# mahdi-slh/DeformContact

Hardware: AMD Instinct MI355X
Metric: M edges/sec fwd+bwd, everyday-deform batch=32 per GPU (encoder hot path) (higher is better)
Workload: dtype f32 (hops, storage, accumulate); wide dense blocks fp16x2-split operands (3 fp16 MFMA products, fp32 accumulate), narrow ones bf16x3-split (6 products); 1 GPU; everyday-deform synthetic, B=32 sample pairs per GPU: soft 32x(1024 v, 6132 e) + rigid 32x(762 v, 4560 e); TAGConv encoder 2 layers/branch, hidden 256, K=3 (configs[1]); edges_per_gpu_step=342144, global_batch=32, settle_steps=150, hipgraph=True, two_stream_branches=True, merged_branches=False, segmented_adjacency_build=True, parallelism=dp1

## Files before the change

### deformcontact_amd/_lib.py

```python
from __future__ import annotations

import ctypes
import os
from ctypes import POINTER, c_char_p, c_float, c_int, c_int32, c_int64, c_void_p

_HERE = os.path.dirname(os.path.abspath(__file__))
SO_PATH = os.path.join(_HERE, "libdeformcontact_hip.so")

_lib = None

_vp = c_void_p
_SIGNATURES = {
    "dc_version": (c_int, []),
    "dc_last_error": (c_char_p, []),
    "dc_stream_capture_id": (c_int64, [_vp]),
    "dc_csr_workspace_bytes": (c_int64, [c_int64, c_int64]),
    "dc_csr_build": (c_int, [_vp, c_int64, c_int64, c_int, c_int, _vp, _vp, _vp, _vp, _vp, _vp,
                             _vp, c_int64, _vp]),
    "dc_graph_workspace_bytes": (c_int64, [c_int64, c_int64]),
    "dc_graph_build": (c_int, [_vp, c_int64, c_int64, c_int, _vp, _vp, _vp, _vp, _vp, _vp, _vp, _vp,
                               _vp, _vp, c_int64, _vp]),
    "dc_graph_build_parts": (c_int, [POINTER(_vp), POINTER(c_int64), POINTER(c_int64), POINTER(c_int64), c_int,
                                     c_int64, c_int, _vp, _vp, _vp, _vp, _vp, _vp, _vp, _vp, _vp, _vp, c_int64,
                                     _vp]),
# ... 12 lines not shown
                                             _vp]),
    "dc_attn_flash_fwd": (c_int, [_vp, c_int64, _vp, _vp, _vp, _vp, _vp, c_int64, c_int64, c_int64, c_int64, _vp,
                                  c_int64, _vp, _vp]),
    "dc_hop_chain_max_nodes": (c_int64, []),
    "dc_hop_chain_lds_request": (c_int64, []),
    "dc_hop_chain_f32": (c_int, [_vp, _vp, _vp, _vp, c_int64, POINTER(c_int64), c_int, _vp, c_int64, c_int64, c_int64,
                                 c_int, c_int, c_int, _vp, c_int, _vp]),
    "dc_spmm_f32_bias_act": (c_int, [_vp, _vp, _vp, _vp, c_int64, _vp, c_int, _vp, c_int64, c_int64, c_int64, _vp]),
    "dc_colsum_workspace_bytes": (c_int64, [c_int64, c_int64, c_int]),
    "dc_mask_colsum_f32": (c_int, [_vp, c_int64, _vp, c_int64, _vp, c_int64, c_int64, c_int64, _vp, c_int64, _vp, c_int,
                                   _vp]),
    "dc_gat_alpha_fwd": (c_int, [_vp, c_int64, _vp, _vp, _vp, _vp, c_int64, c_int64, _vp]),
    "dc_gat_alpha_bwd": (c_int, [_vp, c_int64, _vp, _vp, _vp, _vp, _vp, c_int64, c_int64, c_int64, _vp, c_int64, _vp, _vp,
                                 c_int, _vp]),
    "dc_spmm_f32_pack": (c_int, [_vp, _vp, _vp, _vp, c_int64, _vp, c_int64, c_int64, c_int64, c_int64, c_int64, _vp]),
    "dc_spmm_f32_window": (c_int, [_vp, _vp, _vp, _vp, c_int64, _vp, c_int64, _vp, c_int64, c_int64,
                                   c_int64, c_int64, _vp]),
    "dc_spmm_f32_rowmax_window": (c_int, [_vp, _vp, _vp, _vp, c_int64, _vp, c_int64, _vp, c_int64, c_int64,
                                          c_int64, _vp, c_int, c_int64, _vp]),
    "dc_tag_grouped_weight_prep": (c_int, [POINTER(_vp), c_int, c_int, c_int64, c_int64, POINTER(_vp),
                                           POINTER(_vp), POINTER(_vp), POINTER(_vp), _vp]),
    "dc_tag_grouped_fwd_h2p": (c_int, [_vp, c_int64, c_int, POINTER(c_int64), POINTER(c_int64), c_int64,
                                       POINTER(_vp), POINTER(_vp), c_int, _vp, c_int64, c_int64, c_int64, _vp,
                                       POINTER(_vp), _vp]),
    "dc_tag_grouped_mask_grad": (c_int, [POINTER(_vp), POINTER(c_int64), c_int, POINTER(c_int64),
                                         POINTER(c_int64), c_int64, _vp, c_int64, _vp, c_int64, c_int64, _vp,
                                         _vp, _vp]),
    "dc_tag_grouped_bwd_dw_workspace_bytes": (c_int64, [POINTER(c_int64), c_int, c_int64, c_int64, c_int]),
    "dc_tag_grouped_bwd_dw_h2": (c_int, [_vp, c_int64, POINTER(_vp), POINTER(c_int64), c_int, c_int,
                                         POINTER(c_int64), POINTER(c_int64), c_int64, POINTER(_vp),
# ... 187 lines not shown
```

### deformcontact_amd/csrc/dc_dense.h

```cpp
#pragma once
#include <stdlib.h>

#include "dc_common.h"

namespace dc {

constexpr int BK = 16;
constexpr int LDK = BK + 4;
constexpr int BN = 128;
constexpr int kMaxSeg = DC_MAX_SEG;

using f32x16 = __attribute__((ext_vector_type(16))) float;
using f16x4 = __attribute__((ext_vector_type(4))) _Float16;
using f16x8 = __attribute__((ext_vector_type(8))) _Float16;
using bf16x4 = __attribute__((ext_vector_type(4))) __bf16;
using bf16x8 = __attribute__((ext_vector_type(8))) __bf16;
using s16x4 = __attribute__((ext_vector_type(4))) short;
typedef __attribute__((address_space(3))) s16x4 lds_s16x4;

__device__ __forceinline__ int lds_row_swz(int row) { return ((row >> 1) & 7) ^ ((row & 1) << 1); }

__device__ __forceinline__ void split1(float x, __bf16 &hi, __bf16 &mid, __bf16 &lo) {
    hi = (__bf16)x;
    const float r = x - (float)hi;
    mid = (__bf16)r;
    const float r2 = r - (float)mid;
    lo = (__bf16)r2;
}

__device__ __forceinline__ void split4_h2(const float4 &v, f16x4 &h, f16x4 &l) {
    const float x[4] = {v.x, v.y, v.z, v.w};
#pragma unroll
    for (int i = 0; i < 4; ++i) {
        const _Float16 a = (_Float16)x[i];
        h[i] = a;
        l[i] = (_Float16)(x[i] - (float)a);
    }
}

template <int ROWB>
__device__ __forceinline__ bf16x8 tr_read(const char *a) {
    const s16x4 lo4 = __builtin_amdgcn_ds_read_tr16_b64_v4i16((lds_s16x4 *)(uintptr_t)(a));
// ... 227 lines not shown
```

### deformcontact_amd/csrc/dc_dense_narrow.hip

```cpp
#include "dc_dense.h"

#ifndef DC_NARROW_ABL
#define DC_NARROW_ABL 0
#endif

namespace dc {

struct NarrowParams {
    const float *x;
    int64_t ld;
    const float *w[kMaxSeg];
    int nseg, fi;
    const float *bias;
    float *out;
    int64_t ldo, N;
    int relu, ntiles;
};

constexpr int kNarrowFo = 256;


template <int KS, int MB>
__global__ void __launch_bounds__(256)
k_fwd_narrow(NarrowParams p) {
    constexpr int TR = 32 * MB;
    constexpr int SROWA = KS * 96 + 16;
    constexpr int PPR = 4 * KS;
    constexpr int TP = TR * PPR, NV = (TP + 255) / 256;
    constexpr int KP = 16 * KS;
    constexpr int kOffStage = ((TR * SROWA + 1023) / 1024) * 1024;
    constexpr int kLdsTiles = kOffStage + TR * 1024, kLdsW = kNarrowFo * (KP + 4) * 4;
    __shared__ __attribute__((aligned(1024))) char lds[kLdsTiles > kLdsW ? kLdsTiles : kLdsW];
    char *const sA = lds;
    float *const so = reinterpret_cast<float *>(lds + kOffStage);
// ... 5 lines not shown
        const int64_t row0 = (int64_t)t * TR;
#pragma unroll
        for (int j = 0; j < NV; ++j) {
            const int q = (int)threadIdx.x + 256 * j;
            if (TP % 256 != 0 && q >= TP) continue;
            const int r = q / PPR, c4 = q - r * PPR;
            int64_t row = row0 + r;
            row = row < p.N ? row : p.N - 1;
            if (DC_NARROW_ABL & 8) xv[j] = f32x4{(float)row, 1.f, 2.f, 3.f};
            else xv[j] = *reinterpret_cast<const f32x4 *>(p.x + row * p.ld + 4 * c4);
        }
    };
    int t = blockIdx.x;
    if (t < p.ntiles) load_tile(t);

    constexpr int WROW = KP + 4;
    {
        float *wi = reinterpret_cast<float *>(lds);
        const int width = p.nseg * p.fi, per4 = kNarrowFo * p.fi / 4;
        constexpr int MAXQ = 8;
        f32x4 wv[kMaxSeg][MAXQ];
#pragma unroll
        for (int s = 0; s < kMaxSeg; ++s)
#pragma unroll
            for (int j = 0; j < MAXQ; ++j) {
                const int q = (int)threadIdx.x + 256 * j;
                if (!(DC_NARROW_ABL & 2) && s < p.nseg && q < per4) wv[s][j] = *reinterpret_cast<const f32x4 *>(p.w[s] + 4 * q);
            }
#pragma unroll
        for (int s = 0; s < kMaxSeg; ++s)
#pragma unroll
            for (int j = 0; j < MAXQ; ++j) {
                const int q = (int)threadIdx.x + 256 * j;
                if (!(DC_NARROW_ABL & 2) && s < p.nseg && q < per4) {
                    int o = (4 * q) / p.fi, f = 4 * q - o * p.fi;
#pragma unroll
                    for (int i = 0; i < 4; ++i) {
                        wi[o * WROW + s * p.fi + f] = wv[s][j][i];
                        if (++f == p.fi) f = 0, ++o;
                    }
                }
            }
        const int padw = KP - width;
        for (int e = threadIdx.x; e < kNarrowFo * padw; e += 256) {
            const int o = e / padw, f = e - o * padw;
            wi[o * WROW + width + f] = 0.f;
        }
    }
    __syncthreads();
    bf16x8 fb[2][KS][3];
#pragma unroll
    for (int nb = 0; nb < 2; ++nb) {
        const float *wr = reinterpret_cast<const float *>(lds) + (64 * wid + 32 * nb + c) * WROW + 8 * h;
#pragma unroll
        for (int ks = 0; ks < KS; ++ks) {
            const f32x4 v0 = *reinterpret_cast<const f32x4 *>(wr + 16 * ks);
            const f32x4 v1 = *reinterpret_cast<const f32x4 *>(wr + 16 * ks + 4);
#pragma unroll
            for (int j = 0; j < 8; ++j) {
                __bf16 hi, mid, lo;
                split1(j < 4 ? v0[j] : v1[j - 4], hi, mid, lo);
                fb[nb][ks][0][j] = hi, fb[nb][ks][1][j] = mid, fb[nb][ks][2][j] = lo;
            }
        }
    }
    __syncthreads();
    float bcol[2];
#pragma unroll
    for (int nb = 0; nb < 2; ++nb) bcol[nb] = p.bias ? p.bias[64 * wid + 32 * nb + c] : 0.f;
    const bool relu = p.relu != 0;

    auto store_tile = [&]() {
#pragma unroll
        for (int j = 0; j < NV; ++j) {
            const int q = (int)threadIdx.x + 256 * j;
            if (TP % 256 != 0 && q >= TP) continue;
            const int r = q / PPR, c4 = q - r * PPR;
            bf16x4 hi, mid, lo;
#pragma unroll
            for (int i = 0; i < 4; ++i) {
                __bf16 a, b, d;
// ... 72 lines not shown
    NarrowParams p = p0;
    p.ntiles = (int)((p.N + 31) / 32);
    const unsigned grid = (unsigned)(p.ntiles < 256 ? p.ntiles : 256);
    DC_LAUNCH((k_fwd_narrow<KS, 1>), dim3(grid), dim3(256), 0, hs, p);
}

}

using namespace dc;

extern "C" int dc_tag_linear_fwd_narrow_ok(int64_t fi, int nseg, int64_t wpad, int64_t Fo) {
    return (Fo == kNarrowFo && nseg >= 1 && nseg <= kMaxSeg && fi >= 1 && fi <= 32 && nseg * fi <= wpad &&
            (wpad == 96 || wpad == 112 || wpad == 128)) ? 1 : 0;
}

extern "C" int dc_tag_linear_fwd_narrow(const float *slab, int64_t ld, const float *const *ws, int nseg, int64_t fi,
                                        const float *bias, int relu, float *out, int64_t ldo, int64_t N, int64_t wpad,
                                        int64_t Fo, dc_stream_t stream) {
    DC_REQUIRE(dc_tag_linear_fwd_narrow_ok(fi, nseg, wpad, Fo),
               "dc_tag_linear_fwd_narrow: needs Fo = 256, a padded reduction of 96 / 112 / 128 >= nseg * fi (got Fo=%lld wpad=%lld "
               "nseg=%d fi=%lld)", (long long)Fo, (long long)wpad, nseg, (long long)fi);
    DC_REQUIRE(N >= 0, "dc_tag_linear_fwd_narrow: negative N");
    if (N == 0) return DC_OK;
    DC_REQUIRE(slab && ws && out && ld >= wpad && ldo >= Fo, "dc_tag_linear_fwd_narrow: null pointer / short leading dimension");
    DC_REQUIRE(ld % 4 == 0 && ldo % 4 == 0 && ((uintptr_t)slab & 15) == 0 && ((uintptr_t)out & 15) == 0,
               "dc_tag_linear_fwd_narrow: rows of the slab and of the output must be 16-byte aligned");
    DC_REQUIRE(N < ((int64_t)1 << 31) - 64, "dc_tag_linear_fwd_narrow: too many rows");
    NarrowParams p{};
    p.x = slab, p.ld = ld, p.nseg = nseg, p.fi = (int)fi, p.bias = bias, p.out = out, p.ldo = ldo, p.N = N, p.relu = relu;
    for (int s = 0; s < nseg; ++s) {
        DC_REQUIRE(ws[s], "dc_tag_linear_fwd_narrow: null weight segment %d", s);
        p.w[s] = ws[s];
    }
    hipStream_t hs = (hipStream_t)stream;
    switch (wpad) {
    case 96: narrow_launch<6>(p, hs); break;
    case 112: narrow_launch<7>(p, hs); break;
    default: narrow_launch<8>(p, hs); break;
    }
    return check_launch("dc_tag_linear_fwd_narrow");
}
```

### deformcontact_amd/csrc/dc_spmm.hip

```cpp
#include <stdlib.h>

#include "dc_common.h"

#pragma clang fp contract(off)

namespace dc {

template <int VEC> struct Vec;
template <> struct Vec<1> { using T = float; };
template <> struct Vec<4> { using T = float4; };

__device__ __forceinline__ float vzero(float) { return 0.0f; }
__device__ __forceinline__ float4 vzero(float4) { return make_float4(0.f, 0.f, 0.f, 0.f); }

__device__ __forceinline__ void vaxpy(float &acc, float w, float v) {
    const float m = w * v;
    acc = acc + m;
}
__device__ __forceinline__ void vaxpy(float4 &acc, float w, const float4 &v) {
    const float mx = w * v.x, my = w * v.y, mz = w * v.z, mw = w * v.w;
    acc.x = acc.x + mx;
    acc.y = acc.y + my;
    acc.z = acc.z + mz;
    acc.w = acc.w + mw;
// ... 101 lines not shown
        ww[0] = row_share_f<0>(my_w), ww[1] = row_share_f<1>(my_w), ww[2] = row_share_f<2>(my_w);
        ww[3] = row_share_f<3>(my_w), ww[4] = row_share_f<4>(my_w), ww[5] = row_share_f<5>(my_w);
        ww[6] = row_share_f<6>(my_w), ww[7] = row_share_f<7>(my_w);
    } else {
        const bool mine = sub < 8 && p + sub < end;
        const int my_s = mine ? other[p + sub] : 0;
        const float my_w = mine ? (w ? w[p + sub] : 1.0f) : 0.0f;
#pragma unroll
        for (int j = 0; j < 8; ++j) {
            s[j] = __shfl(my_s, j, L);
            ww[j] = __shfl(my_w, j, L);
        }
    }
}

template <int VEC, int L, int U>
__global__ void __launch_bounds__(256)
k_spmm_sub(const int32_t *__restrict__ ptr, const int32_t *__restrict__ other,
           const float *__restrict__ w, const float *__restrict__ x, int64_t ldx,
           const float *addend, int64_t ldadd, float *y, int64_t ldy,
           int64_t N, int F, int src_off, float *self_dst = nullptr, int pad_beg = 0, int pad_end = 0) {
    using V = typename Vec<VEC>::T;
    constexpr int kRows = 256 / L;
    const unsigned lb = xcd_remap(blockIdx.x, gridDim.x);
    const int64_t row = (int64_t)lb * kRows + threadIdx.x / L;
    if (row >= N) return;
    const int sub = threadIdx.x % L;
    const int beg = ptr[row], end = ptr[row + 1];
    if (self_dst) {
        for (int c = sub; c < F; c += L) self_dst[row * ldy + c] = x[row * ldx + c];
        for (int c = pad_beg + sub; c < pad_end; c += L) self_dst[row * ldy + c] = 0.f;
    }

    for (int c0 = 0; c0 < F; c0 += L * VEC) {
        const int c = c0 + sub * VEC;
        const bool act = c < F;
        V acc = (addend && act) ? *reinterpret_cast<const V *>(addend + row * ldadd + c) : vzero(V{});
        for (int p = beg; p < end; p += U) {
            int s[U];
// ... 14 lines not shown
                const bool ok = act && p + j < end;
                v[j] = ok ? *reinterpret_cast<const V *>(x + (int64_t)(s[j] - src_off) * ldx + c) : vzero(V{});
            }
#pragma unroll
            for (int j = 0; j < U; ++j)
                if (p + j < end) vaxpy(acc, ww[j], v[j]);
        }
        if (act) *reinterpret_cast<V *>(y + row * ldy + c) = acc;
    }
}

template <int VEC, int L, int U>
static void launch_sub(const int32_t *ptr, const int32_t *other, const float *w, const float *x,
                       int64_t ldx, const float *addend, int64_t ldadd, float *y, int64_t ldy,
                       int64_t N, int F, int src_off, hipStream_t stream, float *self_dst = nullptr,
                       int pad_beg = 0, int pad_end = 0) {
    constexpr int kRows = 256 / L;
    const unsigned grid = (unsigned)((N + kRows - 1) / kRows);
    DC_LAUNCH((k_spmm_sub<VEC, L, U>), dim3(grid), dim3(256), 0, stream, ptr, other, w, x,
                       ldx, addend, ldadd, y, ldy, N, F, src_off, self_dst, pad_beg, pad_end);
}

static inline bool aligned16(const void *p) { return ((uintptr_t)p & 15) == 0; }

__device__ __forceinline__ float bf16_to_f32(uint16_t h) { return __uint_as_float((uint32_t)h << 16); }

struct Bf16x8 { uint4 q; };
__device__ __forceinline__ void unpack8(const uint4 &q, float (&v)[8]) {
    const uint32_t d[4] = {q.x, q.y, q.z, q.w};
#pragma unroll
    for (int i = 0; i < 4; ++i) {
        v[2 * i] = __uint_as_float(d[i] << 16);
        v[2 * i + 1] = __uint_as_float(d[i] & 0xffff0000u);
    }
}
// ... 300 lines not shown
    DC_REQUIRE(ptr && x && y, "dc_spmm_f32_bias_act: null ptr/x/y");
    DC_REQUIRE(N < (int64_t)INT32_MAX / 4 && F < (1 << 24) && ldx >= F && ldy >= F && x != y,
               "dc_spmm_f32_bias_act: bad sizes / aliasing");
    const bool vec4 = (F % 4 == 0) && (ldx % 4 == 0) && (ldy % 4 == 0) && aligned16(x) && aligned16(y) &&
                      (!bias || aligned16(bias));
    const unsigned grid = (unsigned)((N + 3) / 4);
    if (vec4)
        DC_LAUNCH((k_spmm_wave<4, 8, false, true>), dim3(grid), dim3(256), 0, stream, ptr, other, w, x, ldx, nullptr,
                  (int64_t)0, y, ldy, N, (int)F, nullptr, 0, 0, bias, relu);
    else
        DC_LAUNCH((k_spmm_wave<1, 8, false, true>), dim3(grid), dim3(256), 0, stream, ptr, other, w, x, ldx, nullptr,
                  (int64_t)0, y, ldy, N, (int)F, nullptr, 0, 0, bias, relu);
    return check_launch("dc_spmm_f32_bias_act");
}

extern "C" int dc_spmm_f32_pack(const int32_t *ptr, const int32_t *other, const float *w, const float *x,
                                int64_t ldx, float *slab, int64_t lds, int64_t N, int64_t F, int64_t width,
                                int64_t wpad, dc_stream_t stream_) {
    hipStream_t stream = (hipStream_t)stream_;
    DC_REQUIRE(N >= 0 && F >= 1 && F <= 32, "dc_spmm_f32_pack: rows of 1..32 floats (got F=%lld)", (long long)F);
    if (N == 0) return DC_OK;
    DC_REQUIRE(ptr && x && slab && (other || true), "dc_spmm_f32_pack: null pointer");
    DC_REQUIRE(N < (int64_t)INT32_MAX / 8 && ldx >= F && width >= 2 * F && wpad >= width && lds >= wpad,
               "dc_spmm_f32_pack: needs ldx >= F, width >= 2 F (block 1 exists), wpad >= width, lds >= wpad");
    DC_REQUIRE((const void *)x != (const void *)slab, "dc_spmm_f32_pack: the slab must not alias x");
    float *y = slab + F;
    if (F > 16)
        launch_sub<1, 32, 8>(ptr, other, w, x, ldx, nullptr, 0, y, lds, N, (int)F, 0, stream, slab, (int)width, (int)wpad);
    else if (F > 8)
        launch_sub<1, 16, 8>(ptr, other, w, x, ldx, nullptr, 0, y, lds, N, (int)F, 0, stream, slab, (int)width, (int)wpad);
    else
        launch_sub<1, 8, 8>(ptr, other, w, x, ldx, nullptr, 0, y, lds, N, (int)F, 0, stream, slab, (int)width, (int)wpad);
    return check_launch("dc_spmm_f32_pack");
}

extern "C" int dc_spmm_f32_window(const int32_t *ptr, const int32_t *other, const float *w,
                                  const float *x, int64_t ldx, const float *addend, int64_t ldadd,
                                  float *y, int64_t ldy, int64_t N, int64_t F, int64_t row_offset,
                                  dc_stream_t stream) {
    DC_REQUIRE(row_offset >= 0 && row_offset < (int64_t)INT32_MAX, "dc_spmm_f32_window: bad row_offset");
    return spmm_f32_impl(ptr, other, w, x, ldx, addend, ldadd, y, ldy, N, F, (int)row_offset, stream);
}

extern "C" int dc_spmm_bf16(const int32_t *ptr, const int32_t *other, const float *w,
                            const uint16_t *x, int64_t ldx, const void *addend, int64_t ldadd,
                            void *y, int64_t ldy, int64_t N, int64_t F, int y_is_f32,
                            dc_stream_t stream_) {
    hipStream_t stream = (hipStream_t)stream_;
// ... 60 lines not shown
```

### deformcontact_amd/ops.py

```python
from __future__ import annotations

import ctypes
import os
from typing import List, Optional

import torch

from . import _lib
from .deferred import resolve
from .graph import GraphIndex, SortedAdjacency, _require_cuda, capture_id, current_stream_ptr


def _rowmajor(t: torch.Tensor, what: str, dtypes=(torch.float32,)) -> int:
    if t.dim() != 2 or t.dtype not in dtypes:
        raise ValueError(f"{what}: expected a 2-D tensor of {dtypes}, got {tuple(t.shape)} {t.dtype}")
    if t.size(1) > 1 and t.stride(1) != 1:
        raise ValueError(f"{what}: innermost dimension must be contiguous")
    return t.stride(0) if t.size(0) > 1 else max(t.stride(0), t.size(1))


def _vp_array(ptrs):
    return (ctypes.c_void_p * len(ptrs))(*ptrs)


# ... 204 lines not shown
        return slab, rowmax
    return None


def _hop_cache_put(g, key, x, slab, rowmax, dev):
    cache = g.__dict__.setdefault("_hop_cache", {})
    if key not in cache:
        while len(cache) >= _HOP_CACHE_ENTRIES:
            cache.pop(next(iter(cache)))
    cache[key] = (slab, rowmax, capture_id(dev), x, x._version)


FUSED_PACK = os.environ.get("DC_FUSED_PACK", "1") != "0"


def _build_input_slab(g: GraphIndex, x: torch.Tensor, k: int, want_rowmax: bool, into=None):
    n, fi = x.shape
    concat, width, wpad = tag_slab_geometry(fi, k)
    dev = x.device
    slab = into[0] if into is not None else _alloc_slab(n, wpad, dev)
    xin = x if (x.dim() == 2 and x.stride(1) == 1) else x.contiguous()
    adj = g.fwd if (g is not None and k >= 1) else None
    if (FUSED_PACK and adj is not None and not want_rowmax and fi <= 32 and not adj.row_offset and g.normalize
            and adj.ptr.numel() == n + 1):
        _lib.check(_lib.lib().dc_spmm_f32_pack(adj.ptr.data_ptr(), adj.other.data_ptr(), adj.w.data_ptr(),
                                               xin.data_ptr(), xin.stride(0), slab.data_ptr(), slab.stride(0), n, fi,
                                               width, wpad, current_stream_ptr(dev)), "dc_spmm_f32_pack")
        for j in range(1, k):
            hop(adj, slab[:, j * fi:(j + 1) * fi], out=slab[:, (j + 1) * fi:(j + 2) * fi], weighted=True)
        return slab, None
    _lib.check(_lib.lib().dc_tag_pack_input(xin.data_ptr(), xin.stride(0), slab.data_ptr(), slab.stride(0), n,
                                            fi, width, wpad, current_stream_ptr(dev)),
               "dc_tag_pack_input")
    rowmax = None
    if want_rowmax:
        rowmax = into[1] if into is not None else torch.empty(n, dtype=torch.float32, device=dev)
    chained_hops(g, slab, fi, k, backward=False, rowmax=rowmax)
    return slab, rowmax


def _tag_uses_h2(fi: int, k: int, fo: Optional[int] = None) -> bool:
    concat, _, wpad = tag_slab_geometry(fi, k)
# ... 103 lines not shown
        return "fp32"
    if _tag_uses_h2(fi, k, None if six else fo):
        return "h2"
    if not tag_slab_geometry(fi, k)[0]:
        return "split"
    return "narrow" if (NARROW_FWD and DENSE_PRODUCTS == 6 and narrow_ok) else "concat"


def _dense_operands(slab: torch.Tensor, fi: int, k: int, concat: bool):
    ld = slab.stride(0)
    if concat:
        return [slab], [ld], slab.size(1), 1
    return [slab[:, j * fi:(j + 1) * fi] for j in range(k + 1)], [ld] * (k + 1), fi, k + 1


def _tag_slab(g, x: torch.Tensor, weights, h2: bool, need_x: bool):
    n, fi = x.shape
    k = len(weights) - 1
    dev = x.device
    wpad = tag_slab_geometry(fi, k)[2]
    slab = _as_slab_block0(x, n, fi, wpad)
    if slab is None and k == 0 and wpad == fi and x.is_contiguous() and x.data_ptr() % 16 == 0:
        slab = x
    rowmax = prepped = None
    if slab is None:
        key = None
        if HOP_CACHE and g is not None and k >= 1 and not need_x:
            key = _hop_cache_key(x, k, wpad, h2)
            hit = _hop_cache_get(g, key, x, dev)
            if hit is not None:
                slab, rowmax = hit
        if slab is None:
            slab, rowmax = _build_input_slab(g, x, k, h2)
            if key is not None:
                _hop_cache_put(g, key, x, slab, rowmax, dev)
    else:
        rowmax = torch.empty(n, dtype=torch.float32, device=dev) if h2 else None
        zeroed = False
        if h2 and g is not None and hop_chain_eligible(g, g.fwd, slab, fi, k):
            fo = weights[0].size(0)
            prepped = _h2_weight_prep(_lib.lib(), [w.contiguous() for w in weights], k, fo, fi,
                                      need_x and fo % 16 == 0, dev, current_stream_ptr(dev), zero=rowmax)
            zeroed = True
        chained_hops(g, slab, fi, k, backward=False, rowmax=rowmax, rowmax_zeroed=zeroed)
    if h2 and k == 0:
        rowmax = rowabsmax(slab)
    return slab, rowmax, prepped

# ... 143 lines not shown
            raise NotImplementedError(f"TAGConv K={k} > {MAX_SEG - 1} is not supported by the fused dense block")
        dev = x.device
        L = _lib.lib()
        st = current_stream_ptr(dev)
        six = next_geom is SIX_PRODUCTS
        if six:
            next_geom = None
        ctx.empty = n == 0
        if ctx.empty:
            ctx.fi, ctx.has_bias = fi, bias is not None
            ctx.save_for_backward(*weights)
            return _tag_out_buffer(next_geom, n, fo, dev)
        concat, width, wpad = tag_slab_geometry(fi, k)
        path = _dense_path(fi, k, fo, six, concat and bool(L.dc_tag_linear_fwd_narrow_ok(fi, k + 1, wpad, fo)))
        need_x = ctx.needs_input_grad[1]
        slab, rowmax, prepped = _tag_slab(g, x, weights, path == "h2", need_x)
        ws = [w.contiguous() for w in weights]
        if concat and path != "narrow":
            ws = [_pack_weights(ws, fo, fi, wpad, st)]
        out = _tag_out_buffer(next_geom, n, fo, dev)
        ldo = out.stride(0)
        b = bias.contiguous() if bias is not None else None
        wt = wt_rowmax = None
        if path == "h2":
            if prepped is None:
                prepped = _h2_weight_prep(L, ws, k, fo, fi, need_x and fo % 16 == 0, dev, st)
            wmax, wimg, wt, wt_rowmax = prepped
            rc = L.dc_tag_linear_fwd_h2p(slab.data_ptr(), slab.stride(0), wimg.data_ptr(), _ptr(b), int(relu),
                                         out.data_ptr(), ldo, n, width, fo, rowmax.data_ptr(), wmax.data_ptr(),
                                         None, 0, st)
        elif path == "narrow":
            rc = L.dc_tag_linear_fwd_narrow(slab.data_ptr(), slab.stride(0), _ptr_array(ws), k + 1, fi, _ptr(b),
                                            int(relu), out.data_ptr(), ldo, n, wpad, fo, st)
        else:
            xs, ldxs, fi_eff, nseg = _dense_operands(slab, fi, k, concat)
            args = (_ptr_array(xs), _i64_array(ldxs), _ptr_array(ws), nseg, _ptr(b), int(relu), out.data_ptr(), ldo,
                    n, fi_eff, fo)
            rc = L.dc_tag_linear_fwd(*args, st) if path == "fp32" else L.dc_tag_linear_fwd_split(*args, DENSE_PRODUCTS, st)
        _lib.check(rc, "dc_tag_linear_fwd")
        ctx.g, ctx.k, ctx.fi, ctx.fo, ctx.has_bias, ctx.relu, ctx.concat, ctx.path = \
            g, k, fi, fo, bias is not None, relu, concat, path
        ctx.params, ctx.bias_param = weights, bias
        ctx.save_for_backward(slab, out if relu else None, rowmax, wt, wt_rowmax, *ws)
        return out

    @staticmethod
    def backward(ctx, gout):
        if ctx.empty:
# ... 1365 lines not shown
```

### include/deformcontact.h

```cpp
#ifndef DEFORMCONTACT_H
#define DEFORMCONTACT_H

#include <stdint.h>

#ifdef __cplusplus
extern "C" {
#endif

#define DC_OK 0
#define DC_EINVAL (-1)
#define DC_ELAUNCH (-2)
#define DC_EWORKSPACE (-3)

typedef void *dc_stream_t;

#define DC_MAX_PARTS 4
#define DC_MAX_GROUPS 4
#define DC_GROUP_ALIGN 256

int dc_version(void);
const char *dc_last_error(void);
int64_t dc_stream_capture_id(dc_stream_t stream);

int64_t dc_csr_workspace_bytes(int64_t E, int64_t N);
// ... 51 lines not shown
int64_t dc_neighbors_compact_workspace_bytes(int64_t ny);
int dc_neighbors_compact(const int32_t *nbr, int cap, const int32_t *counts, int64_t ny, int query_row,
                         int64_t *edge_index, int64_t num_edges, void *workspace, int64_t workspace_bytes,
                         dc_stream_t stream);

int dc_hash_i64(const int64_t *v, int64_t n, uint64_t *out, dc_stream_t stream);

int dc_spmm_f32(const int32_t *ptr, const int32_t *other, const float *w, const float *x,
                int64_t ldx, const float *addend, int64_t ldadd, float *y, int64_t ldy,
                int64_t N, int64_t F, dc_stream_t stream);

int dc_spmm_f32_pack(const int32_t *ptr, const int32_t *other, const float *w, const float *x, int64_t ldx,
                     float *slab, int64_t lds, int64_t N, int64_t F, int64_t width, int64_t wpad,
                     dc_stream_t stream);

int dc_spmm_f32_window(const int32_t *ptr, const int32_t *other, const float *w, const float *x,
                       int64_t ldx, const float *addend, int64_t ldadd, float *y, int64_t ldy,
                       int64_t N, int64_t F, int64_t row_offset, dc_stream_t stream);
int dc_spmm_f32_rowmax_window(const int32_t *ptr, const int32_t *other, const float *w, const float *x,
                              int64_t ldx, const float *addend, int64_t ldadd, float *y, int64_t ldy,
                              int64_t N, int64_t F, float *rowmax, int mode, int64_t row_offset,
                              dc_stream_t stream);

int dc_spmm_bf16(const int32_t *ptr, const int32_t *other, const float *w, const uint16_t *x,
                 int64_t ldx, const void *addend, int64_t ldadd, void *y, int64_t ldy, int64_t N,
                 int64_t F, int y_is_f32, dc_stream_t stream);

int dc_spmm_f32_rowmax(const int32_t *ptr, const int32_t *other, const float *w, const float *x,
                       int64_t ldx, const float *addend, int64_t ldadd, float *y, int64_t ldy,
                       int64_t N, int64_t F, float *rowmax, int mode, dc_stream_t stream);
// ... 30 lines not shown
                      int nseg, const float *bias, int relu, float *out, int64_t ldo,
                      int64_t N, int64_t Fi, int64_t Fo, dc_stream_t stream);

int dc_tag_linear_bwd_dx(const float *g, int64_t ldg, const float *out_for_mask, int64_t ldo,
                         const float *const *ws, int nseg, float *const *gxs,
                         const int64_t *ldgxs, int64_t N, int64_t Fi, int64_t Fo,
                         dc_stream_t stream);

int dc_tag_linear_fwd_split(const float *const *xs, const int64_t *ldxs, const float *const *ws,
                            int nseg, const float *bias, int relu, float *out, int64_t ldo,
                            int64_t N, int64_t Fi, int64_t Fo, int products, dc_stream_t stream);
int dc_tag_linear_fwd_narrow_ok(int64_t fi, int nseg, int64_t wpad, int64_t Fo);
int dc_tag_linear_fwd_narrow(const float *slab, int64_t ld, const float *const *ws, int nseg, int64_t fi,
                             const float *bias, int relu, float *out, int64_t ldo, int64_t N, int64_t wpad,
                             int64_t Fo, dc_stream_t stream);
int64_t dc_tag_linear_bwd_dx_split_workspace_bytes(int64_t Fi, int64_t Fo, int nseg);
int dc_tag_linear_bwd_dx_split(const float *g, int64_t ldg, const float *out_for_mask,
                               int64_t ldo, const float *const *ws, int nseg, float *const *gxs,
                               const int64_t *ldgxs, void *workspace, int64_t workspace_bytes,
                               int64_t N, int64_t Fi, int64_t Fo, int products, dc_stream_t stream);

int64_t dc_tag_linear_bwd_dw_workspace_bytes(int64_t N, int64_t Fi, int64_t Fo, int nseg);
int dc_tag_linear_bwd_dw(const float *g, int64_t ldg, const float *out_for_mask, int64_t ldo,
                         const float *const *xs, const int64_t *ldxs, int nseg,
                         float *const *gws, int ngw, int64_t gw_cols, float *gbias,
                         int accumulate, void *partials, int64_t partials_bytes, int64_t N,
                         int64_t Fi, int64_t Fo, dc_stream_t stream);
int dc_tag_linear_bwd_dw_split(const float *g, int64_t ldg, const float *out_for_mask,
                               int64_t ldo, const float *const *xs, const int64_t *ldxs, int nseg,
                               float *const *gws, int ngw, int64_t gw_cols, float *gbias,
// ... 230 lines not shown
```

Measured before the change: 553.4 M edges/s.

## Precompute narrow-layer bf16x3 weight fragments inside the fused SpMM pack kernel

Extra blocks are appended to the SpMM pack launch to split the narrow layer's weights into bf16 hi/mid/lo MFMA fragment images once per forward. The narrow dense kernel then loads these prebuilt fragments straight into registers, skipping the per-block LDS staging, the two barriers and the repeated splitting. This removes duplicated weight preparation across every output tile block. The cost is a temporary allocation per call and a few extra blocks in the SpMM launch. If the hop cache returns a slab, the image is never built and the old in-kernel path runs.

```diff
diff --git a/deformcontact_amd/_lib.py b/deformcontact_amd/_lib.py
--- a/deformcontact_amd/_lib.py
+++ b/deformcontact_amd/_lib.py
@@ -50,6 +50,11 @@
     "dc_gat_alpha_bwd": (c_int, [_vp, c_int64, _vp, _vp, _vp, _vp, _vp, c_int64, c_int64, c_int64, _vp, c_int64, _vp, _vp,
                                  c_int, _vp]),
     "dc_spmm_f32_pack": (c_int, [_vp, _vp, _vp, _vp, c_int64, _vp, c_int64, c_int64, c_int64, c_int64, c_int64, _vp]),
+    "dc_spmm_f32_pack_wfrag": (c_int, [_vp, _vp, _vp, _vp, c_int64, _vp, c_int64, c_int64, c_int64, c_int64, c_int64,
+                                       POINTER(_vp), c_int, _vp, _vp]),
+    "dc_tag_narrow_wfrag_bytes": (c_int64, [c_int64]),
+    "dc_tag_linear_fwd_narrow_wfrag": (c_int, [_vp, c_int64, POINTER(_vp), c_int, c_int64, _vp, c_int, _vp, c_int64,
+                                               c_int64, c_int64, c_int64, _vp, _vp]),
     "dc_spmm_f32_window": (c_int, [_vp, _vp, _vp, _vp, c_int64, _vp, c_int64, _vp, c_int64, c_int64,
                                    c_int64, c_int64, _vp]),
     "dc_spmm_f32_rowmax_window": (c_int, [_vp, _vp, _vp, _vp, c_int64, _vp, c_int64, _vp, c_int64, c_int64,
diff --git a/deformcontact_amd/csrc/dc_dense.h b/deformcontact_amd/csrc/dc_dense.h
--- a/deformcontact_amd/csrc/dc_dense.h
+++ b/deformcontact_amd/csrc/dc_dense.h
@@ -26,6 +26,43 @@
     mid = (__bf16)r;
     const float r2 = r - (float)mid;
     lo = (__bf16)r2;
+}
+
+constexpr int kNarrowFo = 256;
+constexpr int64_t narrow_wfrag_bytes(int KS) { return (int64_t)4 * 2 * KS * 3 * 64 * 16; }
+__device__ __forceinline__ int64_t narrow_wfrag_offset(int wn, int ks, int KS, int pl, int lane) {
+    return ((((int64_t)wn * KS + ks) * 3 + pl) * 64 + lane) * 16;
+}
+
+struct WFragJob {
+    const float *w[kMaxSeg];
+    int nseg, fi, ks;
+    char *img;
+    unsigned first_block;
+};
+
+__device__ __forceinline__ void narrow_wfrag_produce(const WFragJob &j, unsigned item) {
+    if (item >= 512u * (unsigned)j.ks) return;
+    const int lane = item & 63, g = (int)(item >> 6), ks = g % j.ks, wn = g / j.ks;
+    const int o = 32 * wn + (lane & 31), k0 = 16 * ks + 8 * (lane >> 5);
+    float v[8];
+#pragma unroll
+    for (int i = 0; i < 8; ++i) {
+        const int k = k0 + i;
+        v[i] = 0.f;
+#pragma unroll
+        for (int s = 0; s < kMaxSeg; ++s)
+            if (s < j.nseg && k >= s * j.fi && k < (s + 1) * j.fi) v[i] = j.w[s][(int64_t)o * j.fi + (k - s * j.fi)];
+    }
+    bf16x8 pl[3];
+#pragma unroll
+    for (int i = 0; i < 8; ++i) {
+        __bf16 hi, mid, lo;
+        split1(v[i], hi, mid, lo);
+        pl[0][i] = hi, pl[1][i] = mid, pl[2][i] = lo;
+    }
+#pragma unroll
+    for (int q = 0; q < 3; ++q) *reinterpret_cast<bf16x8 *>(j.img + narrow_wfrag_offset(wn, ks, j.ks, q, lane)) = pl[q];
 }
 
 __device__ __forceinline__ void split4_h2(const float4 &v, f16x4 &h, f16x4 &l) {
diff --git a/deformcontact_amd/csrc/dc_dense_narrow.hip b/deformcontact_amd/csrc/dc_dense_narrow.hip
--- a/deformcontact_amd/csrc/dc_dense_narrow.hip
+++ b/deformcontact_amd/csrc/dc_dense_narrow.hip
@@ -15,9 +15,8 @@
     float *out;
     int64_t ldo, N;
     int relu, ntiles;
+    const char *wfrag;
 };
-
-constexpr int kNarrowFo = 256;
 
 
 template <int KS, int MB>
@@ -53,57 +52,67 @@
     int t = blockIdx.x;
     if (t < p.ntiles) load_tile(t);
 
-    constexpr int WROW = KP + 4;
-    {
-        float *wi = reinterpret_cast<float *>(lds);
-        const int width = p.nseg * p.fi, per4 = kNarrowFo * p.fi / 4;
-        constexpr int MAXQ = 8;
-        f32x4 wv[kMaxSeg][MAXQ];
-#pragma unroll
-        for (int s = 0; s < kMaxSeg; ++s)
-#pragma unroll
-            for (int j = 0; j < MAXQ; ++j) {
-                const int q = (int)threadIdx.x + 256 * j;
-                if (!(DC_NARROW_ABL & 2) && s < p.nseg && q < per4) wv[s][j] = *reinterpret_cast<const f32x4 *>(p.w[s] + 4 * q);
+    bf16x8 fb[2][KS][3];
+    if (p.wfrag) {
+#pragma unroll
+        for (int nb = 0; nb < 2; ++nb)
+#pragma unroll
+            for (int ks = 0; ks < KS; ++ks)
+#pragma unroll
+                for (int pl = 0; pl < 3; ++pl)
+                    fb[nb][ks][pl] = *reinterpret_cast<const bf16x8 *>(p.wfrag + narrow_wfrag_offset(2 * wid + nb, ks, KS, pl, lane));
+    } else {
+        constexpr int WROW = KP + 4;
+        {
+            float *wi = reinterpret_cast<float *>(lds);
+            const int width = p.nseg * p.fi, per4 = kNarrowFo * p.fi / 4;
+            constexpr int MAXQ = 8;
+            f32x4 wv[kMaxSeg][MAXQ];
+#pragma unroll
+            for (int s = 0; s < kMaxSeg; ++s)
+#pragma unroll
+                for (int j = 0; j < MAXQ; ++j) {
+                    const int q = (int)threadIdx.x + 256 * j;
+                    if (!(DC_NARROW_ABL & 2) && s < p.nseg && q < per4) wv[s][j] = *reinterpret_cast<const f32x4 *>(p.w[s] + 4 * q);
+                }
+#pragma unroll
+            for (int s = 0; s < kMaxSeg; ++s)
+#pragma unroll
+                for (int j = 0; j < MAXQ; ++j) {
+                    const int q = (int)threadIdx.x + 256 * j;
+                    if (!(DC_NARROW_ABL & 2) && s < p.nseg && q < per4) {
+                        int o = (4 * q) / p.fi, f = 4 * q - o * p.fi;
+#pragma unroll
+                        for (int i = 0; i < 4; ++i) {
+                            wi[o * WROW + s * p.fi + f] = wv[s][j][i];
+                            if (++f == p.fi) f = 0, ++o;
+                        }
+                    }
+                }
+            const int padw = KP - width;
+            for (int e = threadIdx.x; e < kNarrowFo * padw; e += 256) {
+                const int o = e / padw, f = e - o * padw;
+                wi[o * WROW + width + f] = 0.f;
             }
-#pragma unroll
-        for (int s = 0; s < kMaxSeg; ++s)
-#pragma unroll
-            for (int j = 0; j < MAXQ; ++j) {
-                const int q = (int)threadIdx.x + 256 * j;
-                if (!(DC_NARROW_ABL & 2) && s < p.nseg && q < per4) {
-                    int o = (4 * q) / p.fi, f = 4 * q - o * p.fi;
-#pragma unroll
-                    for (int i = 0; i < 4; ++i) {
-                        wi[o * WROW + s * p.fi + f] = wv[s][j][i];
-                        if (++f == p.fi) f = 0, ++o;
-                    }
+        }
+        __syncthreads();
+#pragma unroll
+        for (int nb = 0; nb < 2; ++nb) {
+            const float *wr = reinterpret_cast<const float *>(lds) + (64 * wid + 32 * nb + c) * WROW + 8 * h;
+#pragma unroll
+            for (int ks = 0; ks < KS; ++ks) {
+                const f32x4 v0 = *reinterpret_cast<const f32x4 *>(wr + 16 * ks);
+                const f32x4 v1 = *reinterpret_cast<const f32x4 *>(wr + 16 * ks + 4);
+#pragma unroll
+                for (int j = 0; j < 8; ++j) {
+                    __bf16 hi, mid, lo;
+                    split1(j < 4 ? v0[j] : v1[j - 4], hi, mid, lo);
+                    fb[nb][ks][0][j] = hi, fb[nb][ks][1][j] = mid, fb[nb][ks][2][j] = lo;
                 }
             }
-        const int padw = KP - width;
-        for (int e = threadIdx.x; e < kNarrowFo * padw; e += 256) {
-            const int o = e / padw, f = e - o * padw;
-            wi[o * WROW + width + f] = 0.f;
-        }
-    }
-    __syncthreads();
-    bf16x8 fb[2][KS][3];
-#pragma unroll
-    for (int nb = 0; nb < 2; ++nb) {
-        const float *wr = reinterpret_cast<const float *>(lds) + (64 * wid + 32 * nb + c) * WROW + 8 * h;
-#pragma unroll
-        for (int ks = 0; ks < KS; ++ks) {
-            const f32x4 v0 = *reinterpret_cast<const f32x4 *>(wr + 16 * ks);
-            const f32x4 v1 = *reinterpret_cast<const f32x4 *>(wr + 16 * ks + 4);
-#pragma unroll
-            for (int j = 0; j < 8; ++j) {
-                __bf16 hi, mid, lo;
-                split1(j < 4 ? v0[j] : v1[j - 4], hi, mid, lo);
-                fb[nb][ks][0][j] = hi, fb[nb][ks][1][j] = mid, fb[nb][ks][2][j] = lo;
-            }
-        }
-    }
-    __syncthreads();
+        }
+        __syncthreads();
+    }
     float bcol[2];
 #pragma unroll
     for (int nb = 0; nb < 2; ++nb) bcol[nb] = p.bias ? p.bias[64 * wid + 32 * nb + c] : 0.f;
@@ -206,9 +215,9 @@
             (wpad == 96 || wpad == 112 || wpad == 128)) ? 1 : 0;
 }
 
-extern "C" int dc_tag_linear_fwd_narrow(const float *slab, int64_t ld, const float *const *ws, int nseg, int64_t fi,
-                                        const float *bias, int relu, float *out, int64_t ldo, int64_t N, int64_t wpad,
-                                        int64_t Fo, dc_stream_t stream) {
+static int fwd_narrow_impl(const float *slab, int64_t ld, const float *const *ws, int nseg, int64_t fi, const float *bias,
+                           int relu, float *out, int64_t ldo, int64_t N, int64_t wpad, int64_t Fo, const void *wfrag,
+                           dc_stream_t stream) {
     DC_REQUIRE(dc_tag_linear_fwd_narrow_ok(fi, nseg, wpad, Fo),
                "dc_tag_linear_fwd_narrow: needs Fo = 256, a padded reduction of 96 / 112 / 128 >= nseg * fi (got Fo=%lld wpad=%lld "
                "nseg=%d fi=%lld)", (long long)Fo, (long long)wpad, nseg, (long long)fi);
@@ -217,9 +226,11 @@
     DC_REQUIRE(slab && ws && out && ld >= wpad && ldo >= Fo, "dc_tag_linear_fwd_narrow: null pointer / short leading dimension");
     DC_REQUIRE(ld % 4 == 0 && ldo % 4 == 0 && ((uintptr_t)slab & 15) == 0 && ((uintptr_t)out & 15) == 0,
                "dc_tag_linear_fwd_narrow: rows of the slab and of the output must be 16-byte aligned");
+    DC_REQUIRE(((uintptr_t)wfrag & 15) == 0, "dc_tag_linear_fwd_narrow: the fragment image must be 16-byte aligned");
     DC_REQUIRE(N < ((int64_t)1 << 31) - 64, "dc_tag_linear_fwd_narrow: too many rows");
     NarrowParams p{};
     p.x = slab, p.ld = ld, p.nseg = nseg, p.fi = (int)fi, p.bias = bias, p.out = out, p.ldo = ldo, p.N = N, p.relu = relu;
+    p.wfrag = (const char *)wfrag;
     for (int s = 0; s < nseg; ++s) {
         DC_REQUIRE(ws[s], "dc_tag_linear_fwd_narrow: null weight segment %d", s);
         p.w[s] = ws[s];
@@ -232,3 +243,19 @@
     }
     return check_launch("dc_tag_linear_fwd_narrow");
 }
+
+extern "C" int dc_tag_linear_fwd_narrow(const float *slab, int64_t ld, const float *const *ws, int nseg, int64_t fi,
+                                        const float *bias, int relu, float *out, int64_t ldo, int64_t N, int64_t wpad,
+                                        int64_t Fo, dc_stream_t stream) {
+    return fwd_narrow_impl(slab, ld, ws, nseg, fi, bias, relu, out, ldo, N, wpad, Fo, nullptr, stream);
+}
+
+extern "C" int dc_tag_linear_fwd_narrow_wfrag(const float *slab, int64_t ld, const float *const *ws, int nseg, int64_t fi,
+                                              const float *bias, int relu, float *out, int64_t ldo, int64_t N, int64_t wpad,
+                                              int64_t Fo, const void *wfrag, dc_stream_t stream) {
+    return fwd_narrow_impl(slab, ld, ws, nseg, fi, bias, relu, out, ldo, N, wpad, Fo, wfrag, stream);
+}
+
+extern "C" int64_t dc_tag_narrow_wfrag_bytes(int64_t wpad) {
+    return (wpad == 96 || wpad == 112 || wpad == 128) ? narrow_wfrag_bytes((int)(wpad / 16)) : 0;
+}
diff --git a/deformcontact_amd/csrc/dc_spmm.hip b/deformcontact_amd/csrc/dc_spmm.hip
--- a/deformcontact_amd/csrc/dc_spmm.hip
+++ b/deformcontact_amd/csrc/dc_spmm.hip
@@ -1,6 +1,6 @@
 #include <stdlib.h>
 
-#include "dc_common.h"
+#include "dc_dense.h"
 
 #pragma clang fp contract(off)
 
@@ -139,15 +139,24 @@
     }
 }
 
-template <int VEC, int L, int U>
+template <int VEC, int L, int U, bool WF = false>
 __global__ void __launch_bounds__(256)
 k_spmm_sub(const int32_t *__restrict__ ptr, const int32_t *__restrict__ other,
            const float *__restrict__ w, const float *__restrict__ x, int64_t ldx,
            const float *addend, int64_t ldadd, float *y, int64_t ldy,
-           int64_t N, int F, int src_off, float *self_dst = nullptr, int pad_beg = 0, int pad_end = 0) {
+           int64_t N, int F, int src_off, float *self_dst = nullptr, int pad_beg = 0, int pad_end = 0,
+           WFragJob wf = WFragJob{}) {
     using V = typename Vec<VEC>::T;
     constexpr int kRows = 256 / L;
-    const unsigned lb = xcd_remap(blockIdx.x, gridDim.x);
+    unsigned nblk = gridDim.x;
+    if constexpr (WF) {
+        if (blockIdx.x >= wf.first_block) {
+            narrow_wfrag_produce(wf, (blockIdx.x - wf.first_block) * 256u + threadIdx.x);
+            return;
+        }
+        nblk = wf.first_block;
+    }
+    const unsigned lb = xcd_remap(blockIdx.x, nblk);
     const int64_t row = (int64_t)lb * kRows + threadIdx.x / L;
     if (row >= N) return;
     const int sub = threadIdx.x % L;
@@ -192,11 +201,18 @@
 static void launch_sub(const int32_t *ptr, const int32_t *other, const float *w, const float *x,
                        int64_t ldx, const float *addend, int64_t ldadd, float *y, int64_t ldy,
                        int64_t N, int F, int src_off, hipStream_t stream, float *self_dst = nullptr,
-                       int pad_beg = 0, int pad_end = 0) {
+                       int pad_beg = 0, int pad_end = 0, const WFragJob *wf = nullptr) {
     constexpr int kRows = 256 / L;
     const unsigned grid = (unsigned)((N + kRows - 1) / kRows);
+    if (wf) {
+        WFragJob job = *wf;
+        job.first_block = grid;
+        DC_LAUNCH((k_spmm_sub<VEC, L, U, true>), dim3(grid + 2u * job.ks), dim3(256), 0, stream, ptr, other, w, x,
+                           ldx, addend, ldadd, y, ldy, N, F, src_off, self_dst, pad_beg, pad_end, job);
+        return;
+    }
     DC_LAUNCH((k_spmm_sub<VEC, L, U>), dim3(grid), dim3(256), 0, stream, ptr, other, w, x,
-                       ldx, addend, ldadd, y, ldy, N, F, src_off, self_dst, pad_beg, pad_end);
+                       ldx, addend, ldadd, y, ldy, N, F, src_off, self_dst, pad_beg, pad_end, WFragJob{});
 }
 
 static inline bool aligned16(const void *p) { return ((uintptr_t)p & 15) == 0; }
@@ -527,9 +543,9 @@
     return check_launch("dc_spmm_f32_bias_act");
 }
 
-extern "C" int dc_spmm_f32_pack(const int32_t *ptr, const int32_t *other, const float *w, const float *x,
-                                int64_t ldx, float *slab, int64_t lds, int64_t N, int64_t F, int64_t width,
-                                int64_t wpad, dc_stream_t stream_) {
+static int spmm_f32_pack_impl(const int32_t *ptr, const int32_t *other, const float *w, const float *x, int64_t ldx,
+                              float *slab, int64_t lds, int64_t N, int64_t F, int64_t width, int64_t wpad,
+                              const WFragJob *wf, dc_stream_t stream_) {
     hipStream_t stream = (hipStream_t)stream_;
     DC_REQUIRE(N >= 0 && F >= 1 && F <= 32, "dc_spmm_f32_pack: rows of 1..32 floats (got F=%lld)", (long long)F);
     if (N == 0) return DC_OK;
@@ -539,12 +555,35 @@
     DC_REQUIRE((const void *)x != (const void *)slab, "dc_spmm_f32_pack: the slab must not alias x");
     float *y = slab + F;
     if (F > 16)
-        launch_sub<1, 32, 8>(ptr, other, w, x, ldx, nullptr, 0, y, lds, N, (int)F, 0, stream, slab, (int)width, (int)wpad);
+        launch_sub<1, 32, 8>(ptr, other, w, x, ldx, nullptr, 0, y, lds, N, (int)F, 0, stream, slab, (int)width, (int)wpad, wf);
     else if (F > 8)
-        launch_sub<1, 16, 8>(ptr, other, w, x, ldx, nullptr, 0, y, lds, N, (int)F, 0, stream, slab, (int)width, (int)wpad);
+        launch_sub<1, 16, 8>(ptr, other, w, x, ldx, nullptr, 0, y, lds, N, (int)F, 0, stream, slab, (int)width, (int)wpad, wf);
     else
-        launch_sub<1, 8, 8>(ptr, other, w, x, ldx, nullptr, 0, y, lds, N, (int)F, 0, stream, slab, (int)width, (int)wpad);
+        launch_sub<1, 8, 8>(ptr, other, w, x, ldx, nullptr, 0, y, lds, N, (int)F, 0, stream, slab, (int)width, (int)wpad, wf);
     return check_launch("dc_spmm_f32_pack");
+}
+
+extern "C" int dc_spmm_f32_pack(const int32_t *ptr, const int32_t *other, const float *w, const float *x,
+                                int64_t ldx, float *slab, int64_t lds, int64_t N, int64_t F, int64_t width,
+                                int64_t wpad, dc_stream_t stream) {
+    return spmm_f32_pack_impl(ptr, other, w, x, ldx, slab, lds, N, F, width, wpad, nullptr, stream);
+}
+
+extern "C" int dc_spmm_f32_pack_wfrag(const int32_t *ptr, const int32_t *other, const float *w, const float *x,
+                                      int64_t ldx, float *slab, int64_t lds, int64_t N, int64_t F, int64_t width,
+                                      int64_t wpad, const float *const *ws, int nseg, void *wfrag, dc_stream_t stream) {
+    DC_REQUIRE(ws && wfrag && ((uintptr_t)wfrag & 15) == 0, "dc_spmm_f32_pack_wfrag: null / misaligned fragment image");
+    DC_REQUIRE(nseg >= 1 && nseg <= kMaxSeg && (int64_t)nseg * F == width && (wpad == 96 || wpad == 112 || wpad == 128),
+               "dc_spmm_f32_pack_wfrag: needs width = nseg * F and a padded reduction of 96 / 112 / 128 (got nseg=%d F=%lld "
+               "width=%lld wpad=%lld)", nseg, (long long)F, (long long)width, (long long)wpad);
+    DC_REQUIRE(N > 0, "dc_spmm_f32_pack_wfrag: no rows, no launch: the image would not be written");
+    WFragJob job{};
+    for (int s = 0; s < nseg; ++s) {
+        DC_REQUIRE(ws[s], "dc_spmm_f32_pack_wfrag: null weight segment %d", s);
+        job.w[s] = ws[s];
+    }
+    job.nseg = nseg, job.fi = (int)F, job.ks = (int)(wpad / 16), job.img = (char *)wfrag;
+    return spmm_f32_pack_impl(ptr, other, w, x, ldx, slab, lds, N, F, width, wpad, &job, stream);
 }
 
 extern "C" int dc_spmm_f32_window(const int32_t *ptr, const int32_t *other, const float *w,
diff --git a/deformcontact_amd/ops.py b/deformcontact_amd/ops.py
--- a/deformcontact_amd/ops.py
+++ b/deformcontact_amd/ops.py
@@ -242,7 +242,16 @@
 FUSED_PACK = os.environ.get("DC_FUSED_PACK", "1") != "0"
 
 
-def _build_input_slab(g: GraphIndex, x: torch.Tensor, k: int, want_rowmax: bool, into=None):
+NARROW_WFRAG = True
+
+
+class _WFragRequest:
+
+    def __init__(self, ws, wpad: int):
+        self.ws, self.wpad, self.image = ws, wpad, None
+
+
+def _build_input_slab(g: GraphIndex, x: torch.Tensor, k: int, want_rowmax: bool, into=None, wfrag=None):
     n, fi = x.shape
     concat, width, wpad = tag_slab_geometry(fi, k)
     dev = x.device
@@ -251,9 +260,16 @@
     adj = g.fwd if (g is not None and k >= 1) else None
     if (FUSED_PACK and adj is not None and not want_rowmax and fi <= 32 and not adj.row_offset and g.normalize
             and adj.ptr.numel() == n + 1):
-        _lib.check(_lib.lib().dc_spmm_f32_pack(adj.ptr.data_ptr(), adj.other.data_ptr(), adj.w.data_ptr(),
-                                               xin.data_ptr(), xin.stride(0), slab.data_ptr(), slab.stride(0), n, fi,
-                                               width, wpad, current_stream_ptr(dev)), "dc_spmm_f32_pack")
+        L = _lib.lib()
+        args = (adj.ptr.data_ptr(), adj.other.data_ptr(), adj.w.data_ptr(), xin.data_ptr(), xin.stride(0),
+                slab.data_ptr(), slab.stride(0), n, fi, width, wpad)
+        if wfrag is not None and n > 0 and wfrag.wpad == wpad and L.dc_tag_narrow_wfrag_bytes(wpad) > 0:
+            image = torch.empty(L.dc_tag_narrow_wfrag_bytes(wpad), dtype=torch.uint8, device=dev)
+            _lib.check(L.dc_spmm_f32_pack_wfrag(*args, _ptr_array(wfrag.ws), k + 1, image.data_ptr(),
+                                                current_stream_ptr(dev)), "dc_spmm_f32_pack_wfrag")
+            wfrag.image = image
+        else:
+            _lib.check(L.dc_spmm_f32_pack(*args, current_stream_ptr(dev)), "dc_spmm_f32_pack")
         for j in range(1, k):
             hop(adj, slab[:, j * fi:(j + 1) * fi], out=slab[:, (j + 1) * fi:(j + 2) * fi], weighted=True)
         return slab, None
@@ -387,7 +403,7 @@
     return [slab[:, j * fi:(j + 1) * fi] for j in range(k + 1)], [ld] * (k + 1), fi, k + 1
 
 
-def _tag_slab(g, x: torch.Tensor, weights, h2: bool, need_x: bool):
+def _tag_slab(g, x: torch.Tensor, weights, h2: bool, need_x: bool, wfrag=None):
     n, fi = x.shape
     k = len(weights) - 1
     dev = x.device
@@ -404,7 +420,7 @@
             if hit is not None:
                 slab, rowmax = hit
         if slab is None:
-            slab, rowmax = _build_input_slab(g, x, k, h2)
+            slab, rowmax = _build_input_slab(g, x, k, h2, wfrag=wfrag)
             if key is not None:
                 _hop_cache_put(g, key, x, slab, rowmax, dev)
     else:
@@ -578,8 +594,9 @@
         concat, width, wpad = tag_slab_geometry(fi, k)
         path = _dense_path(fi, k, fo, six, concat and bool(L.dc_tag_linear_fwd_narrow_ok(fi, k + 1, wpad, fo)))
         need_x = ctx.needs_input_grad[1]
-        slab, rowmax, prepped = _tag_slab(g, x, weights, path == "h2", need_x)
         ws = [w.contiguous() for w in weights]
+        wfrag = _WFragRequest(ws, wpad) if (path == "narrow" and NARROW_WFRAG) else None
+        slab, rowmax, prepped = _tag_slab(g, x, weights, path == "h2", need_x, wfrag)
         if concat and path != "narrow":
             ws = [_pack_weights(ws, fo, fi, wpad, st)]
         out = _tag_out_buffer(next_geom, n, fo, dev)
@@ -594,8 +611,9 @@
                                          out.data_ptr(), ldo, n, width, fo, rowmax.data_ptr(), wmax.data_ptr(),
                                          None, 0, st)
         elif path == "narrow":
-            rc = L.dc_tag_linear_fwd_narrow(slab.data_ptr(), slab.stride(0), _ptr_array(ws), k + 1, fi, _ptr(b),
-                                            int(relu), out.data_ptr(), ldo, n, wpad, fo, st)
+            rc = L.dc_tag_linear_fwd_narrow_wfrag(slab.data_ptr(), slab.stride(0), _ptr_array(ws), k + 1, fi, _ptr(b),
+                                                  int(relu), out.data_ptr(), ldo, n, wpad, fo,
+                                                  _ptr(wfrag.image) if wfrag is not None else None, st)
         else:
             xs, ldxs, fi_eff, nseg = _dense_operands(slab, fi, k, concat)
             args = (_ptr_array(xs), _i64_array(ldxs), _ptr_array(ws), nseg, _ptr(b), int(relu), out.data_ptr(), ldo,
diff --git a/include/deformcontact.h b/include/deformcontact.h
--- a/include/deformcontact.h
+++ b/include/deformcontact.h
@@ -89,6 +89,10 @@
                      float *slab, int64_t lds, int64_t N, int64_t F, int64_t width, int64_t wpad,
                      dc_stream_t stream);
 
+int dc_spmm_f32_pack_wfrag(const int32_t *ptr, const int32_t *other, const float *w, const float *x, int64_t ldx,
+                           float *slab, int64_t lds, int64_t N, int64_t F, int64_t width, int64_t wpad,
+                           const float *const *ws, int nseg, void *wfrag, dc_stream_t stream);
+
 int dc_spmm_f32_window(const int32_t *ptr, const int32_t *other, const float *w, const float *x,
                        int64_t ldx, const float *addend, int64_t ldadd, float *y, int64_t ldy,
                        int64_t N, int64_t F, int64_t row_offset, dc_stream_t stream);
@@ -149,6 +153,10 @@
 int dc_tag_linear_fwd_narrow(const float *slab, int64_t ld, const float *const *ws, int nseg, int64_t fi,
                              const float *bias, int relu, float *out, int64_t ldo, int64_t N, int64_t wpad,
                              int64_t Fo, dc_stream_t stream);
+int64_t dc_tag_narrow_wfrag_bytes(int64_t wpad);
+int dc_tag_linear_fwd_narrow_wfrag(const float *slab, int64_t ld, const float *const *ws, int nseg, int64_t fi,
+                                   const float *bias, int relu, float *out, int64_t ldo, int64_t N, int64_t wpad,
+                                   int64_t Fo, const void *wfrag, dc_stream_t stream);
 int64_t dc_tag_linear_bwd_dx_split_workspace_bytes(int64_t Fi, int64_t Fo, int nseg);
 int dc_tag_linear_bwd_dx_split(const float *g, int64_t ldg, const float *out_for_mask,
                                int64_t ldo, const float *const *ws, int nseg, float *const *gxs,
```

New measurement: 560.3 M edges/s, median of 6. Within noise of the previous version (+1.3%).
